# e271828e/Flight.jl

Hardware: AMD Instinct MI355X
Metric: aircraft-steps/sec (higher is better)
Workload: dtype f64

## Files before the change

flight.jl_amd/csrc/c172_duo_device.hpp:

```cpp
#pragma once
#include "c172_device.hpp"

namespace fbd {

#if defined(FB_STAMP) && defined(FB_DUO_TIMELINE)
__device__ unsigned long long g_duo_t0[2];
__device__ __forceinline__ void duo_mark(int role, int k) {
    __builtin_amdgcn_sched_barrier(0);
    if (blockIdx.x == 0 && (threadIdx.x & 255) == 0) {
        const unsigned long long t = __builtin_amdgcn_s_memtime();
        if (k == 0) g_duo_t0[role - 1] = t;
        else if (g_duo_t0[role - 1] != 0) { g_stamp_acc[(role == 1 ? 0 : 16) + k] += t - g_duo_t0[role - 1]; g_stamp_cnt[(role == 1 ? 0 : 16) + k] += 1; }
    }
    __builtin_amdgcn_sched_barrier(0);
}
#define DUO_MARK(role, k) duo_mark(role, k)
#else
#define DUO_MARK(role, k) do { } while (0)
#endif

enum { DUO_PT_T = 0, DUO_PT_V = 1, DUO_PT_X = 2,
       DUO_PT_R = 0, DUO_PT_A = 1, DUO_PT_W = 2,
       DUO_NPT = 3 };
constexpr int XD_FP = 0, XD_TAUP = 3, XD_HROT = 6, XD_RHO = 7, XD_HO = 8, XD_ROWS = 9;
constexpr int XD_VP = XD_FP;
constexpr int DUO_TAP_THETA_ROW = 0, DUO_TAP_WX_ROW = 2, DUO_TAP_VD_ROW = 5, DUO_TAP_EAS_ROW = 7, DUO_TAP_ALPHA_ROW = 8, DUO_TAP_LAT_ROW = 10;

enum {
    KC_P_PROP_HI = KC_HELPERS_END, KC_P_PROP_RSTEP,
    KC_P_WGS_A, KC_P_PROP_RX, KC_P_PROP_RZ,
    KC_P_INV_R, KC_P_INV_SQRT_GR, KC_P_INV_TWO_PI, KC_P_0P1, KC_P_PROP_JXX,
    KC_P_FRC_KP, KC_P_FRC_KI, KC_P_INV_W_IDLE, KC_P_INV_W_RATED, KC_P_INV_P_STD,
    KC_P_N2_LO, KC_P_N2_RSTEP, KC_P_D9_LO, KC_P_D9_RSTEP, KC_P_M9_LO, KC_P_M9_RSTEP,
    KC_P_INV_RHO_STD, KC_P_F_DIFF, KC_P_F_RICH, KC_P_5EM3, KC_P_SQRT_T_STD, KC_P_P_RATED, KC_P_TAU_FRC, KC_P_INV_J, KC_P_INV_M_FUEL,
    KC_P_F_LEAN,
    KC_COUNT
};
FB_KC(KC_P_PROP_HI, 1.5); FB_KC(KC_P_PROP_RSTEP, (PR_NJ - 1) / (1.5 - 0.0));
static_assert(PR_NJ == PR_NM, "one reciprocal step serves both axes of the propeller table");
FB_KC(KC_P_WGS_A, wgs::a); FB_KC(KC_P_PROP_RX, c172::prop_r[0]); FB_KC(KC_P_PROP_RZ, c172::prop_r[2]);
FB_KC(KC_P_INV_R, 1 / isa::R); FB_KC(KC_P_INV_SQRT_GR, 1 / 20.046795704052055); FB_KC_RCP(KC_P_INV_TWO_PI, 2 * PI); FB_KC(KC_P_0P1, 0.1);
FB_KC(KC_P_PROP_JXX, c172::prop_Jxx); FB_KC(KC_P_FRC_KP, 5.0); FB_KC(KC_P_FRC_KI, 200.0);
FB_KC_RCP(KC_P_INV_W_IDLE, c172::w_idle); FB_KC_RCP(KC_P_INV_W_RATED, c172::w_rated); FB_KC_RCP(KC_P_INV_P_STD, isa::p_std);
FB_KC(KC_P_N2_LO, 0.667); FB_KC(KC_P_N2_RSTEP, (2 - 1) / (1.0 - 0.667));
FB_KC(KC_P_D9_LO, 0.441); FB_KC(KC_P_D9_RSTEP, (9 - 1) / (1.0 - 0.441));
FB_KC(KC_P_M9_LO, 0.401); FB_KC(KC_P_M9_RSTEP, (9 - 1) / (0.936 - 0.401));
FB_KC(KC_P_INV_RHO_STD, 1 / isa::rho_std); FB_KC(KC_P_F_DIFF, c172::f_rich - c172::f_lean); FB_KC(KC_P_F_RICH, c172::f_rich); FB_KC(KC_P_5EM3, 5e-3);
FB_KC(KC_P_SQRT_T_STD, isa_sqrt_T_std); FB_KC(KC_P_P_RATED, c172::P_rated); FB_KC(KC_P_TAU_FRC, 0.01 * c172::P_rated / c172::w_rated);
FB_KC_RCP(KC_P_INV_J, c172::J_eng + c172::prop_Jxx); FB_KC_RCP(KC_P_INV_M_FUEL, c172::m_full - c172::m_res);
FB_KC(KC_P_F_LEAN, c172::f_lean);

template <int KIN, int ROLE, class In, class Emit, class XV, class KP = KLit>
__device__ __forceinline__ int32_t rhs_duo(const XV& x, int stall, int eng_state, const In& in, const Env& env, const Tables& T, const Emit& emit, StepAux& aux,
                                           const KP& K = KP{}) {
    using namespace c172;
    static_assert(ROLE == 1 || ROLE == 2, "role P or role D");
    static_assert(KIN == FB_KIN_WA || KIN == FB_KIN_ECEF || KIN == FB_KIN_NED, "kinematic mechanisation");
    int32_t st = 0;
    constexpr int KX = FB_X_Q_WB;
    constexpr bool X = Emit::x2;
    auto gkp = [&](int off) -> gk_cptr { return T.gk + off; };
    auto atan2m = [&](double y, double x0) -> double { return atan2_step(y, x0, T.rk + LDS_ATAN, K); };
    auto atan2p = [&](double y, double x0) -> double { return atan2_step<true>(y, x0, T.rk + LDS_ATAN, K); };

    const double h_e = x[KIN == FB_KIN_WA ? KX + 8 : (KIN == FB_KIN_ECEF ? KX + 7 : KX + 5)];
    if (!(h_e >= H_MIN)) st |= FB_ST_ALT_RANGE;
    [[maybe_unused]] quat q_ew = {1, 0, 0, 0};
    [[maybe_unused]] double dq12 = 0, dq13 = 0, dq24 = 0, dq34 = 0;
    [[maybe_unused]] double ned_cla = 1, pos0 = 0, pos1 = 0, pos2 = 0;
    v3 n_e;
    if constexpr (KIN == FB_KIN_WA) {
        q_ew = {x[KX + 4], x[KX + 5], x[KX + 6], x[KX + 7]};
        dq12 = 2 * q_ew.w * q_ew.x; dq13 = 2 * q_ew.w * q_ew.y;
        dq24 = 2 * q_ew.x * q_ew.z; dq34 = 2 * q_ew.y * q_ew.z;
        n_e = {-(dq24 + dq13), -(dq34 - dq12), -(1 - 2 * (q_ew.x * q_ew.x + q_ew.y * q_ew.y))};
    } else if constexpr (KIN == FB_KIN_ECEF) {
        pos0 = x[KX + 4]; pos1 = x[KX + 5]; pos2 = x[KX + 6];
        n_e = {pos0, pos1, pos2};
    } else {
        pos0 = x[KX + 3]; pos1 = x[KX + 4];
        double sla, slo, clo;
        sincos_step(pos0, sla, ned_cla); sincos_step(pos1, slo, clo);
        n_e = {ned_cla * clo, ned_cla * slo, sla};
    }
    const v3 r_p = {prop_r[0], prop_r[1], prop_r[2]};

    if constexpr (ROLE == 1) {
        lds_cptr PT = T.lds + LDS_PISTON;
        lds_cptr RPT = T.rk + LDS_PISTON;
        const double w_eng = x[FB_X_ENG_OMEGA];
        const double x_frc = x[FB_X_ENG_FRC], x_idle = x[FB_X_ENG_IDLE], x_fuel = x[FB_X_FUEL];
        {
            double pin_w = w_eng, pin_f = x_frc, pin_i = x_idle, pin_u = x_fuel, pin_h = h_e;
            asm volatile("" : "+v"(pin_w), "+v"(pin_f), "+v"(pin_i), "+v"(pin_u), "+v"(pin_h));
            if constexpr (KIN == FB_KIN_WA) {
                double pin_q0 = q_ew.w, pin_q1 = q_ew.x, pin_q2 = q_ew.y, pin_q3 = q_ew.z;
                asm volatile("" : "+v"(pin_q0), "+v"(pin_q1), "+v"(pin_q2), "+v"(pin_q3));
            } else {
                double pin_p0 = pos0, pin_p1 = pos1, pin_p2 = pos2;
                asm volatile("" : "+v"(pin_p0), "+v"(pin_p1), "+v"(pin_p2));
            }
        }
        emit.xpub(DUO_PT_R);
        if constexpr (X) __builtin_amdgcn_s_setprio(0);
        double lat, lon;
        const double h_o = h_e - geoid_height<true>(T, n_e, lat, lon, K);
        if (!(h_o >= H_MIN)) st |= FB_ST_ALT_RANGE;
        if constexpr (X) {
            if (emit.tap) {
                const double ll[2] = {KIN == FB_KIN_NED ? pos0 : lat, KIN == FB_KIN_NED ? pos1 : lon};
                emit.template tap_rows<2>(DUO_TAP_LAT_ROW, ll);
            }
        }
        DUO_MARK(1, 1);
        double T_air, p_air, lnp_air;
        const double h_gp = h_o * kc<KC_P_WGS_A>(K) / (kc<KC_P_WGS_A>(K) + h_o);
        isa_data<true>(h_gp, env.T_sl, env.p_sl, T_air, p_air, lnp_air, st, K);
        const double rs_T = rsqrt(T_air), i_T = rs_T * rs_T;
        const double rho = (p_air * kc<KC_P_INV_R>(K)) * i_T;
        const double i_a_snd = kc<KC_P_INV_SQRT_GR>(K) * rs_T;
        DUO_MARK(1, 2);
        emit.xput(XD_RHO, rho); emit.xput(XD_HO, h_o);
        DUO_MARK(1, 11);
        emit.xpub(DUO_PT_A);
        emit.xwait(DUO_PT_V);
        DUO_MARK(1, 3);

        const double w_prop = w_eng;
        const v3 v_p = {emit.xget(XD_VP), emit.xget(XD_VP + 1), emit.xget(XD_VP + 2)};
        const double v_J = norm(v_p, K);
        const double J_adv = kc<KC_TWO_PI>(K) * v_J / (fmax(fabs(w_prop), 1.0) * prop_d);
        const double Mt = fabs(w_prop) * (prop_d / 2) * i_a_snd;
        const loc lj = range_locate(0.0, kc<KC_P_PROP_HI>(K), kc<KC_P_PROP_RSTEP>(K), PR_NJ, J_adv, true);
        const loc lm = range_locate(0.0, kc<KC_P_PROP_HI>(K), kc<KC_P_PROP_RSTEP>(K), PR_NM, Mt, true);
        const double w00 = (1 - lj.w) * (1 - lm.w), w01 = (1 - lj.w) * lm.w, w10 = lj.w * (1 - lm.w), w11 = lj.w * lm.w;
        gk_cptr g00 = T.gk + LDS_PROP + (lj.i + PR_NJ * lm.i) * PR_NC;
        auto coef = [&](int cidx) {
            return (w00 * g00[cidx] + w01 * g00[PR_NJ * PR_NC + cidx]) + (w10 * g00[PR_NC + cidx] + w11 * g00[PR_NJ * PR_NC + PR_NC + cidx]);
        };
        const double C_Fx = coef(0), C_Mx = coef(1), C_Fz_a = coef(2), C_Mz_a = coef(3);
        double a_p = 0, b_p = 0;
        if (!(v_J < kc<KC_P_0P1>(K))) {
            a_p = atan2m(v_p.z, v_p.x);
            b_p = atan2p(v_p.y, sqrt(v_p.x * v_p.x + v_p.z * v_p.z, K));
        }
// ... 219 lines not shown
        v3 d_e;
        const v3 g_c_c = gravity_com(q_eb, r_bc, n_e, h_e, R_N, R_E, i_RN, i_RE, st, d_e);
        const v3 w_ie_b = earth_rate_b(q_eb);

        DUO_MARK(2, 7);
        emit.xwait(DUO_PT_A);
        const double rho = emit.xget(XD_RHO), h_o = emit.xget(XD_HO);
        if (!(h_o >= H_MIN)) st |= FB_ST_ALT_RANGE;
        if (!(h_o * wgs::a < 84852.0 * (wgs::a + h_o))) st |= FB_ST_ISA_RANGE;
        const double q_dyn = 0.5 * rho * (TAS * TAS);
        if constexpr (X) { if (emit.tap) { const double e1[1] = {TAS * sqrt(rho / isa::rho_std)}; emit.template tap_rows<1>(DUO_TAP_EAS_ROW, e1); } }
        const double p_nd = w_wb_b.x * b * i2V, q_nd = w_wb_b.y * c * i2V, r_nd = w_wb_b.z * b * i2V;
        const double dh_nd = (h_o - env.h_trn) / b;
        const loc l_ge = grid_locate<13, true, AUX_GE>(A + AT_GE_K, RA + AT_GE_K, dh_nd, true, true, gkp(LDS_AERO + AT_GE_K), T.gk);
        auto S_ = [&](int k) -> double { return T.gk[LDS_AERO + AT_SCALARS + k]; };
        if constexpr (X) {
            ac.cy_in = S_(AS_CY_DR) * x2_dr + S_(AS_CY_DA) * x2_da;
            ac.cl_in = S_(AS_CL_DE) * x2_de;
            ac.croll_in = S_(AS_Cl_DA) * x2_da + S_(AS_Cl_DR) * x2_dr;
            ac.cn_in = S_(AS_CN_DR) * x2_dr + S_(AS_CN_DA) * x2_da;
        }
        const double C_D = ac.cd_in + lerp1(A + AT_CD_GE_V, l_ge) * cd_al + cd_be;
        const double C_Y = ac.cy_in + cy_be + cy_p * p_nd + cy_r * r_nd;
        const double C_L = lerp1(A + AT_CL_GE_V, l_ge) * cl_al + ac.cl_in + S_(AS_CL_Q) * q_nd + S_(AS_CL_ALPHA_DOT) * ad_nd;
        const double C_l = ac.croll_in + S_(AS_Cl_BETA) * be + S_(AS_Cl_P) * p_nd + cl_r * r_nd;
        const double C_m = ac.cm_in + S_(AS_CM_ALPHA) * al + S_(AS_CM_Q) * q_nd + S_(AS_CM_ALPHA_DOT) * ad_nd;
        const double C_n = ac.cn_in + S_(AS_CN_BETA) * be + S_(AS_CN_P) * p_nd + S_(AS_CN_R) * r_nd;
        const double qS = q_dyn * S;
        const v3 F_s = {qS * -C_D, qS * C_Y, qS * -C_L};
        const v3 F_a = {cos_al * F_s.x - sin_al * F_s.z, F_s.y, sin_al * F_s.x + cos_al * F_s.z};
        const v3 tau_a = {qS * (C_l * b), qS * (C_m * c), qS * (C_n * b)};
        aux.alpha = alpha;
        aux.wow = 0;
        aux.crash = 0;
        if (!(fmin(h_o - env.h_trn, h_e - H_MIN) > 10.0)) st |= FB_ST_INTERNAL_REDO;
        auto Jmul = [&](v3 v) { return v3{Jxx * v.x + Jxy * v.y + Jxz * v.z, Jxy * v.x + Jyy * v.y + Jyz * v.z, Jxz * v.x + Jyz * v.y + Jzz * v.z}; };
        const v3 v_ec_c = v_eb_b + cross(w_eb_b, r_bc);
        const v3 w_ic_c = w_ie_b + w_eb_b;
        v3 T0 = tau_a - cross(r_bc, F_a) - Jmul(cross(w_ie_b, w_eb_b)) - cross(w_ic_c, Jmul(w_ic_c));
        v3 A0 = iM * F_a + g_c_c - cross(w_eb_b + 2.0 * w_ie_b, v_ec_c);
        const double c11 = Jyy * Jzz - Jyz * Jyz, c12 = Jyz * Jxz - Jxy * Jzz, c13 = Jxy * Jyz - Jyy * Jxz;
        const double c22 = Jxx * Jzz - Jxz * Jxz, c23 = Jxy * Jxz - Jxx * Jyz, c33 = Jxx * Jyy - Jxy * Jxy;
        const double idet = 1 / (Jxx * c11 + Jxy * c12 + Jxz * c13);
        double i11 = c11 * idet, i12 = c12 * idet, i13 = c13 * idet, i22 = c22 * idet, i23 = c23 * idet, i33 = c33 * idet;
        double wy = w_ic_c.y, wz = w_ic_c.z;
        asm volatile("" : "+v"(T0.x), "+v"(T0.y), "+v"(T0.z), "+v"(A0.x), "+v"(A0.y), "+v"(A0.z));
        asm volatile("" : "+v"(i11), "+v"(i12), "+v"(i13), "+v"(i22), "+v"(i23), "+v"(i33), "+v"(wy), "+v"(wz));
        DUO_MARK(2, 8);
        emit.xwait(DUO_PT_W);
        DUO_MARK(2, 9);
        const v3 F_p = {emit.xget(XD_FP), emit.xget(XD_FP + 1), emit.xget(XD_FP + 2)};
        const v3 tau_pb = {emit.xget(XD_TAUP), emit.xget(XD_TAUP + 1), emit.xget(XD_TAUP + 2)};
        const double h_rot = emit.xget(XD_HROT);
        {
            double p0 = F_p.x, p1 = F_p.y, p2 = F_p.z, p3 = tau_pb.x, p4 = tau_pb.y, p5 = tau_pb.z, p6 = h_rot;
            asm volatile("" : "+v"(p0), "+v"(p1), "+v"(p2), "+v"(p3), "+v"(p4), "+v"(p5), "+v"(p6));
        }
        emit.xpub(DUO_PT_X);
        const v3 rw = (T0 + tau_pb) - cross(r_bc, F_p) - v3{0.0, wz * h_rot, -(wy * h_rot)};
        const v3 wd = {i11 * rw.x + i12 * rw.y + i13 * rw.z, i12 * rw.x + i22 * rw.y + i23 * rw.z, i13 * rw.x + i23 * rw.y + i33 * rw.z};
        const v3 vd_b = (A0 + iM * F_p) - cross(wd, r_bc);
        DUO_MARK(2, 10);
        const double kd6[6] = {wd.x, wd.y, wd.z, vd_b.x, vd_b.y, vd_b.z};
        emit_rows<6>(emit, FB_X_OMEGA_EB_B, kd6);
        DUO_MARK(2, 11);
        return st;
    }
}

}
```

flight.jl_amd/csrc/c172_kernels.hpp:

```cpp
#pragma once
#include "c172_device.hpp"
#include "c172x_ctl_device.hpp"
#include "c172_duo_device.hpp"

namespace fbd {

template <bool FAST>
__device__ __forceinline__ void ground_common(quat q_eb, quat q_en, GroundCommon& c) {
    c.q_en = q_en;
    if constexpr (FAST) {
        auto rot_z = [](quat q) { return v3{(2 * q.y) * q.w - (2 * q.z) * (-q.x), (2 * q.z) * q.y - (2 * q.x) * q.w, 1 + ((2 * q.x) * (-q.x) - (2 * q.y) * q.y)}; };
        c.ks_e = rot_z(q_eb);
        c.ut_e = rot_z(c.q_en);
    } else {
        c.ks_e = qrot(q_eb, v3{0, 0, 1});
        c.ut_e = qrot(c.q_en, v3{0, 0, 1});
    }
    c.ut_ks = dot(c.ut_e, c.ks_e);
    if constexpr (FAST) {
        const bool lo = c.ut_ks < 0.5 - 1e-7, hi = c.ut_ks > 0.5 + 1e-7;
        c.tilt_crash = lo;
        if (__builtin_amdgcn_ballot_w64(!lo && !hi) != 0) {
            const double a = acos(fmax(fmin(c.ut_ks, 1.0), -1.0));
            if (!lo && !hi) c.tilt_crash = a * (180 / PI) > 60;
// ... 848 lines not shown
    auto TAP = [&](int k) { return t0[(int64_t)k * n]; };
    auto XS = [&](int k) { return xs[SV::row(k) * B]; };
    CtlIn v;
    {
        const gcptr u0 = (gcptr)(uintptr_t)A.cu + i;
        v.lat = TAP(DUO_TAP_LAT); v.lon = TAP(DUO_TAP_LON); v.EAS = TAP(DUO_TAP_EAS); v.phi = TAP(DUO_TAP_PHI);
        if constexpr (HALF == CTL_HALF_LON) {
            v.theta = TAP(DUO_TAP_THETA); v.clm = -TAP(DUO_TAP_VD); v.alpha = TAP(DUO_TAP_ALPHA);
            v.w_wb_b = {0.0, TAP(DUO_TAP_WY), TAP(DUO_TAP_WZ)};
            v.pos[0] = TAP(DUO_TAP_POS + 0); v.pos[2] = TAP(DUO_TAP_POS + 2); v.cmd[0] = TAP(DUO_TAP_CMD + 0); v.cmd[2] = TAP(DUO_TAP_CMD + 2);
            v.pos[1] = v.pos[3] = v.cmd[1] = v.cmd[3] = 0; v.chi = 0; v.beta = 0;
        } else {
            v.chi = TAP(DUO_TAP_CHI); v.beta = TAP(DUO_TAP_BETA);
            v.theta = 0; v.clm = 0;
            v.w_wb_b = {TAP(DUO_TAP_WX), 0.0, 0.0};
            v.pos[1] = TAP(DUO_TAP_POS + 1); v.pos[3] = TAP(DUO_TAP_POS + 3); v.cmd[1] = TAP(DUO_TAP_CMD + 1); v.cmd[3] = TAP(DUO_TAP_CMD + 3);
            v.pos[0] = v.pos[2] = v.cmd[0] = v.cmd[2] = 0; v.alpha = 0;
        }
#pragma unroll
        for (int k = 0; k < FB_NCU; k++) lu[k] = u0[(int64_t)k * n];
    }
    v.h_e = h_e;
    v.w_eb_b = {XS(FB_X_OMEGA_EB_B), XS(FB_X_OMEGA_EB_B + 1), XS(FB_X_OMEGA_EB_B + 2)};
    v.alpha_filt = XS(FB_X_ALPHA_FILT); v.beta_filt = XS(FB_X_BETA_FILT);
    v.n_eng = XS(FB_X_ENG_OMEGA) / c172::w_rated;
    v.on_gnd = false;
    const CtlMemHalfT<gptr, HALF> M = {(gptr)(uintptr_t)A.cu + i, (gptr)(uintptr_t)A.cs + i, n, lu};
    FB_HALF_STAMP(HALF, HALF == CTL_HALF_LON ? 22 : 16);
    gdc_update(M, v);
    FB_HALF_STAMP(HALF, HALF == CTL_HALF_LON ? 23 : 17);
    const CtlTabT<gcptr> tab = ctl_tab((gcptr)(uintptr_t)A.gains, A.off, v.EAS, v.h_e);
    if constexpr (HALF == CTL_HALF_LON) {
        ctl_lon<true>(tab, M, A.dT, v, (int)M.U(FB_CU_LON_MODE_REQ));
        FB_HALF_STAMP(HALF, 24);
        return {clampd(M.S(FB_CS_THROTTLE_CMD), 0, 1), clampd(M.S(FB_CS_ELEVATOR_CMD), -1, 1)};
    } else {
        const int lat_req = (int)M.U(FB_CU_LAT_MODE_REQ);
        LatGains G;
        G.P = {0, 0, 0, 0};
        ctl_lat<true>(tab, M, A.dT, v, lat_req, G);
        FB_HALF_STAMP(HALF, 19);
        return {clampd(M.S(FB_CS_AILERON_CMD), -1, 1), clampd(M.S(FB_CS_RUDDER_CMD), -1, 1)};
    }
}

constexpr int DUO_B = 256;
constexpr int DUO_NP = 4, DUO_ND = 17;
constexpr int DUO_NPL = 0;
constexpr int DUO_NDL_WA = 13;
constexpr int DUO_NDL_X = 14;
template <int KIN, bool X> constexpr int duo_ndl() { return (KIN == FB_KIN_WA && !X) ? DUO_NDL_WA : (X ? DUO_NDL_X : DUO_ND); }
static_assert(DUO_NDL_WA >= 1 && DUO_NDL_WA <= DUO_ND && DUO_NDL_X >= 1 && DUO_NDL_X <= DUO_ND, "");
template <int KIN, bool X, bool PERENV> constexpr int duo_nk() { return (KIN == FB_KIN_WA && !X && !PERENV) ? (int)KC_COUNT : 0; }
template <int NK>
struct DuoK {
    double r[NK];
    template <int I> static constexpr bool resident() { return I < NK; }
    template <int I> __device__ __forceinline__ double get() const { if constexpr (I < NK) return r[I]; else return KC<I>::v; }
    template <int I = 0> __device__ __forceinline__ void init() {
        if constexpr (I < NK) { double c = KC<I>::v; asm volatile("" : "+v"(c)); r[I] = c; init<I + 1>(); }
    }
};
template <> struct DuoK<0> : KLit { __device__ __forceinline__ void init() {} };
struct InputsDuoP {
    double throttle, mixture;
    int ui;
    __device__ __forceinline__ double get_throttle() const { return throttle; }
    __device__ __forceinline__ double get_mixture() const { return mixture; }
};
struct InputsDuoD {
    static constexpr bool pld_precomputed = true, aero_precomputed = true;
    lds_cptr pld_l;
    const double* aero_g;
    int64_t n;
    int ui;
    __device__ __forceinline__ double get_pld_M() const { return pld_l[0]; }
    __device__ __forceinline__ double get_pld_Mr(int k) const { return pld_l[(1 + k) * DUO_B]; }
    __device__ __forceinline__ double get_pld_J(int k) const { return pld_l[(4 + k) * DUO_B]; }
    static constexpr int SUMS_ROWS = 10;
    __device__ __forceinline__ void fetch_pld_raw(double (&v)[10]) const {
#pragma unroll
        for (int k = 0; k < 10; k++) v[k] = aero_g[(int64_t)k * n];
    }
    __device__ __forceinline__ void fetch_aero(AeroC& c) const {
        double v[DUO_NCONST];
        fetch_aero_raw(v);
        aero_from_raw(v, c);
    }
    __device__ __forceinline__ void fetch_aero_raw(double (&v)[DUO_NCONST]) const {
#pragma unroll
        for (int k = 0; k < DUO_NCONST; k++) v[k] = aero_g[(int64_t)k * n];
    }
    __device__ __forceinline__ static void aero_from_raw(const double (&v)[DUO_NCONST], AeroC& c) {
        c.cd_in = v[0]; c.cd_df = v[1]; c.cy_in = v[2]; c.cl_in = v[3]; c.cl_df = v[4]; c.croll_in = v[5]; c.cm_in = v[6]; c.cn_in = v[7];
        c.l_df4 = {(int)v[8], v[9]}; c.l_df2 = {(int)v[10], v[11]};
    }
};
struct InputsDuoDX : InputsDuoD {
    double pldv[10];
    __device__ __forceinline__ double get_pld_M() const { return pldv[0]; }
    __device__ __forceinline__ double get_pld_Mr(int k) const { return pldv[1 + k]; }
    __device__ __forceinline__ double get_pld_J(int k) const { return pldv[4 + k]; }
};
#ifdef FB_DUO_SYNC_DEBUG
__device__ unsigned g_duo_sync_dbg[40];
#endif
struct DuoSync {
    volatile __attribute__((address_space(3))) int* mine;
    volatile __attribute__((address_space(3))) int* other;
    int base;
    int failed;
};
template <bool GLOBAL = false>
FBD void duo_publish(DuoSync& sy, int k) {
    if constexpr (GLOBAL) asm volatile("s_waitcnt vmcnt(0) lgkmcnt(0)" ::: "memory");
    else asm volatile("s_waitcnt lgkmcnt(0)" ::: "memory");
    *sy.mine = sy.base + k + 1;
    asm volatile("" ::: "memory");
}
FBD void duo_wait(DuoSync& sy, int k) {
#if defined(FB_STAMP) && defined(FB_DUO_WAITPROF)
    const unsigned long long t0 = __builtin_amdgcn_s_memtime();
#endif
    const int c = sy.base + k + 1;
    asm volatile("" ::: "memory");
    int spins = 0;
#pragma unroll 1
    while (__builtin_amdgcn_readfirstlane(*sy.other) < c) {
        __builtin_amdgcn_s_sleep(1);
#ifdef FB_DUO_SYNC_DEBUG
        if (++spins > (1 << 10)) {
            sy.failed = 1;
            if ((threadIdx.x & 63) == 0 && atomicAdd(&g_duo_sync_dbg[0], 1u) < 7) {
                const unsigned q = atomicAdd(&g_duo_sync_dbg[1], 4u);
                g_duo_sync_dbg[2 + q] = blockIdx.x; g_duo_sync_dbg[3 + q] = threadIdx.x; g_duo_sync_dbg[4 + q] = c; g_duo_sync_dbg[5 + q] = *sy.other;
            }
            break;
        }
#else
        if (++spins > (1 << 20)) { sy.failed = 1; break; }
#endif
    }
    asm volatile("" ::: "memory");
#if defined(FB_STAMP) && defined(FB_DUO_WAITPROF)
    const unsigned long long t1 = __builtin_amdgcn_s_memtime();
    if (blockIdx.x == 0 && (threadIdx.x == 0 || threadIdx.x == DUO_B)) {
        const int q = k + (threadIdx.x ? 8 : 0);
        g_stamp_acc[q] += t1 - t0; g_stamp_cnt[q] += 1;
    }
#endif
}

template <int ROLE, bool X = false, int NDL = DUO_ND>
struct DuoEmit {
    static constexpr int role = ROLE;
    static constexpr bool x2 = X;
    typedef void batched_tag;
    using SV = StateLds<DUO_B, false>;
    lds_cptr xs_l;
    lds_ptr xwr_l;
    lds_ptr acc_l;
    double* acc_r;
    lds_ptr xch_l;
    lds_ptr xov_l;
    double eb, ee, em;
    bool last;
    int t;
    DuoSync* sync;
    bool tap;
    int64_t ai;
    const double* xn_r = nullptr;
    template <int N>
    __device__ __forceinline__ void tap_rows(int k0, const double (&v)[N]) const {
        const kargs_cptr ka = kernarg();
        double* const g = ka->duo_tap + ai;
        const int64_t n = ka->n;
#pragma unroll
        for (int e = 0; e < N; e++) g[(int64_t)(k0 + e) * n] = v[e];
    }
    __device__ __forceinline__ static constexpr bool owned(int j) {
        if (SV::skip(j)) return false;
        const int r = SV::row(j);
        return ROLE == 1 ? (r >= 2 && r <= 5) : (r < 2 || r >= 6);
    }
    __device__ __forceinline__ static constexpr int slot(int r) { return ROLE == 1 ? r - 2 : (r < 2 ? r : r - 4); }
    __device__ __forceinline__ double aget(int r) const {
        if (ROLE == 1 && slot(r) >= DUO_NPL) return acc_r[slot(r) - DUO_NPL];
        if (ROLE == 2 && slot(r) >= NDL) return acc_r[slot(r) - NDL];
        return acc_l[slot(r) * DUO_B + t];
    }
    __device__ __forceinline__ void aset(int r, double v) const {
        if (ROLE == 1 && slot(r) >= DUO_NPL) acc_r[slot(r) - DUO_NPL] = v;
        else if (ROLE == 2 && slot(r) >= NDL) acc_r[slot(r) - NDL] = v;
        else acc_l[slot(r) * DUO_B + t] = v;
    }
    __device__ __forceinline__ void operator()(int j, double kj) const {
        static_assert(ROLE == 1 || ROLE == 2, "");
        const int r = SV::row(j), idx = r * DUO_B + t;
        const double xs = (ROLE == 1 && !X) ? xn_r[slot(r)] : xs_l[idx];
        const double A = __builtin_fma(eb, kj, aget(r));
        aset(r, A * em);
        xwr_l[idx] = __builtin_fma(ee, last ? A : kj, xs);
    }
    template <int NE>
    __device__ __forceinline__ void batch(int j0, const double (&k)[NE]) const {
        double xs[NE], A[NE];
#pragma unroll
        for (int e = 0; e < NE; e++) { const int r = SV::row(j0 + e); xs[e] = (ROLE == 1 && !X) ? xn_r[slot(r)] : xs_l[r * DUO_B + t]; A[e] = aget(r); }
#pragma unroll
        for (int e = 0; e < NE; e++) A[e] = __builtin_fma(eb, k[e], A[e]);
#pragma unroll
        for (int e = 0; e < NE; e++) {
            const int r = SV::row(j0 + e);
            aset(r, A[e] * em);
            xwr_l[r * DUO_B + t] = __builtin_fma(ee, last ? A[e] : k[e], xs[e]);
        }
    }
    __device__ __forceinline__ void xput(int k, double v) const { if (k < 6) xov_l[k * DUO_B + t] = v; else xch_l[(k - 6) * DUO_B + t] = v; }
    __device__ __forceinline__ double xget(int k) const { return k < 6 ? xov_l[k * DUO_B + t] : xch_l[(k - 6) * DUO_B + t]; }
    __device__ __forceinline__ void xpub(int k) const { if (X && tap && ROLE == 1) duo_publish<true>(*sync, k); else duo_publish<false>(*sync, k); }
    __device__ __forceinline__ void xwait(int k) const { duo_wait(*sync, k); }
};
constexpr bool duo_rows_ok() {
    int np = 0, nd = 0;
    bool seen_p[DUO_NP] = {}, seen_d[DUO_ND] = {};
    for (int j = 0; j < FB_NX; j++) {
        if (StateLds<DUO_B, false>::skip(j)) { if (DuoEmit<1>::owned(j) || DuoEmit<2>::owned(j)) return false; continue; }
        const int r = StateLds<DUO_B, false>::row(j);
        if (DuoEmit<1>::owned(j) == DuoEmit<2>::owned(j)) return false;
        if (DuoEmit<1>::owned(j)) { const int k = DuoEmit<1>::slot(r); if (k < 0 || k >= DUO_NP || seen_p[k]) return false; seen_p[k] = true; np++; }
        else { const int k = DuoEmit<2>::slot(r); if (k < 0 || k >= DUO_ND || seen_d[k]) return false; seen_d[k] = true; nd++; }
    }
    return np == DUO_NP && nd == DUO_ND;
}
static_assert(duo_rows_ok(), "k_step_duo: row ownership / stage-sum slots");
static_assert(DuoEmit<1>::owned(FB_X_FUEL) && DuoEmit<1>::owned(FB_X_ENG_OMEGA) && DuoEmit<2>::owned(FB_X_Q_WB) && DuoEmit<2>::owned(FB_X_V_EB_B + 2),
              "rhs_duo emits the engine and fuel rows in role P, everything else in role D");
enum { DUO_F_RUN = 1, DUO_F_ZERO_ACC = 2, DUO_F_ENG_SHIFT = 2, DUO_F_CTL = 16 };
enum { DUO_C_EXIT = 4, DUO_C_TAP = 8, DUO_C_CMD = 16 };
constexpr int DUO_PT_U = DUO_NPT, DUO_PT_F = DUO_NPT;
#if defined(FB_STAMP) && defined(FB_DUO_PHASES)
#define DUO_PHASE(k) do { if (blockIdx.x == 0 && threadIdx.x == 256) { __builtin_amdgcn_s_waitcnt(0); g_stamp_acc[8 + (k)] = __builtin_amdgcn_s_memtime(); g_stamp_cnt[8 + (k)] += 1; } } while (0)
#else
#define DUO_PHASE(k) do { } while (0)
#endif
template <int KIN, bool X = false, bool PERENV = false>
__global__ __launch_bounds__(2 * DUO_B) void k_step_duo(KArgs a, int nsteps) {
    constexpr int B = DUO_B, NR = FB_NX - 6, NP = DUO_NP, ND = DUO_ND;
    constexpr int NPT = X ? DUO_NPT + 2 : DUO_NPT;
    constexpr int NAL = FB_ACT_BRAKE_LEFT;
    using SV = StateLds<B, false>;
    __shared__ double lds[AT_SIZE + PT_SIZE];
    __shared__ double rk[LDS_RK_DOUBLES];
    __shared__ double xs_l[NR * B];
    __shared__ double xc_l[NR * B];
    constexpr int DUO_NDL = duo_ndl<KIN, X>();
    __shared__ double accd_l[DUO_NDL * B];
    __shared__ double accp_l[(DUO_NPL > 0 ? DUO_NPL : 1) * B];
    __shared__ double pld_l[10 * B];
    __shared__ double xch_l[(XD_ROWS - 6) * B];
    __shared__ int flags_l[B];
    __shared__ int dst_l[B];
    constexpr bool ENV_LDS = PERENV && (KIN == FB_KIN_WA || X);
    __shared__ double envd_l[ENV_LDS ? 4 * B : 1];
    static_assert(LDS_RK_DOUBLES >= LDS_ATAN + ATAN_N + 2, "room for the control words behind the atan table");
    int* ctrl_l = (int*)&rk[LDS_ATAN + ATAN_N];
// ... 128 lines not shown
            if (c & DUO_C_EXIT) break;
            const bool run = f & DUO_F_RUN;
            const int eng = (f >> DUO_F_ENG_SHIFT) & 3;
            if (f & DUO_F_ZERO_ACC) {
#pragma unroll
                for (int k = 0; k < NP - DUO_NPL; k++) acc_r[k] = 0.0;
#pragma unroll
                for (int k = 0; k < DUO_NPL; k++) accp_l[k * B + t] = 0.0;
            }
            const int stg = c & 3;
            if (!X && stg == 0) {
#pragma unroll
                for (int k = 0; k < NP; k++) xn_r[k] = xs_l[(2 + k) * B + t];
            }
            const StageK sk = stage_k(stg);
            int lds_off = 0;
            asm volatile("" : "+s"(lds_off));
            const Tables T = {(lds_cptr)lds + lds_off, a.egm96, (lds_cptr)rk + lds_off, (gk_cptr)a.tables + lds_off};
            [[maybe_unused]] const bool tap = X && (c & DUO_C_TAP);
            if constexpr (X) { if (sums_for != stg || (c & DUO_C_CMD)) form_sums(stg, lds_off); }
            if (__builtin_amdgcn_ballot_w64(run) != 0) {
                if (run) {
                    StepAux aux;
                    InputsDuoP inl = in;
                    if constexpr (X) {
                        double z = z0;
                        asm volatile("" : "+v"(z));
                        const double ms = act_stage_mc(stg, z);
                        inl.throttle = clampd(act_stage_pos(xa[FB_ACT_THROTTLE], ca[FB_ACT_THROTTLE], ms), 0.0, 1.0);
                    }
                    DUO_MARK(1, 12);
                    asm volatile("" : "+v"(inl.throttle), "+v"(inl.mixture));
                    const DuoEmit<1, X> emit = {(lds_cptr)xs_l, sk.xwr_l, (lds_ptr)accp_l, acc_r, (lds_ptr)xch_l, (lds_ptr)xc_l + 15 * B, sk.eb, sk.ee, sk.em, sk.last, t, &sy,
                                                tap, i, xn_r};
                    if constexpr (X) {
                        if (tap) {
                            static_assert(DUO_TAP_CMD == DUO_TAP_POS + 4, "positions, then commands");
                            const double pc[8] = {clampd(xa[0], 0.0, 1.0), clampd(xa[1], -1.0, 1.0), clampd(xa[2], -1.0, 1.0), clampd(xa[3], -1.0, 1.0), ca[0], ca[1], ca[2], ca[3]};
                            emit.template tap_rows<8>(DUO_TAP_POS, pc);
                        }
                    }
                    const SV xv = {sk.xrd_l + t + lds_off};
#if defined(FB_DUO_ONLY) && FB_DUO_ONLY == 2
                    emit.xpub(DUO_PT_R);
                    emit.xput(XD_RHO, 1.1); emit.xput(XD_HO, 1000.0);
                    emit.xpub(DUO_PT_A);
                    emit.xwait(DUO_PT_V);
                    emit.xput(XD_FP, 900.0); emit.xput(XD_FP + 1, 0.0); emit.xput(XD_FP + 2, 0.0);
                    emit.xput(XD_TAUP, -150.0); emit.xput(XD_TAUP + 1, 0.0); emit.xput(XD_TAUP + 2, 700.0); emit.xput(XD_HROT, 80.0);
                    emit.xpub(DUO_PT_W);
                    emit.xwait(DUO_PT_X);
                    (void)xv; (void)aux; (void)inl;
#else
                    rhs_duo<KIN, 1>(xv, 0, eng, inl, env_p, T, emit, aux, kres);
#endif
                    if constexpr (X) {
                        if (sk.last) {
                            double z = z0;
                            asm volatile("" : "+v"(z));
                            const double P = 1 - z + z * z / 2 - z * z * z / 6 + z * z * z * z / 24;
#pragma unroll
                            for (int k = 0; k < NAL; k++) xa[k] = ca[k] + (xa[k] - ca[k]) * P;
                        }
                    }
                }
            } else duo_publish(sy, DUO_PT_W);
            if constexpr (X) {
                if (tap) {
                    DUO_MARK(1, 13);
                    duo_wait(sy, DUO_PT_U);
                    DUO_MARK(1, 14);
                    const bool ctl = flags_l[t] & DUO_F_CTL;
                    __builtin_amdgcn_s_setprio(X2_LON_PRIO);
#ifdef FB_X2_SKIP_LON
                    if (false) {
#else
                    if (ctl) {
#endif
                        const Ctl2 co = ctl_half(std::integral_constant<int, CTL_HALF_LON>{}, i);
                        ca[FB_ACT_THROTTLE] = co.c0; ca[FB_ACT_ELEVATOR] = co.c1;
                    }
                    DUO_MARK(1, 7);
                    __builtin_amdgcn_s_setprio(0);
                    duo_publish<true>(sy, DUO_PT_F);
                }
                if (tap) sums_for = -1;
                else {
                    __builtin_amdgcn_s_setprio(X2_SPEC_PRIO);
                    form_sums((stg + 1) & 3, lds_off);
                    __builtin_amdgcn_s_setprio(0);
                }
            }
            sy.base += NPT;
        }
        if constexpr (X) {
            const int d = dst_l[t];
            if (valid && (d & D_ACTIVE) && !(d & D_HANDOFF)) {
                bool bad = false;
#pragma unroll
                for (int k = 0; k < NAL; k++) { bad = bad || !isfinite(xa[k]); a.x[(int64_t)(X2_ACT + k) * a.n + i] = xa[k]; }
                if (bad) atomicOr(&a.status[i], (int32_t)FB_ST_NAN);
            }
        }
        if (__builtin_amdgcn_ballot_w64(sy.failed != 0) != 0 && valid) atomicOr(&a.status[i], (int32_t)FB_ST_NAN);
        return;
    }
    InputsDuoD in;
    in.pld_l = (lds_cptr)pld_l + t; in.aero_g = a.duo_pld + (valid ? i : 0); in.n = a.n; in.ui = 0;
    double accd_r[ND > DUO_NDL ? ND - DUO_NDL : 1];
#pragma unroll
    for (int k = 0; k < (ND > DUO_NDL ? ND - DUO_NDL : 1); k++) accd_r[k] = 0.0;
    {
        int stall = 0, eng = 0;
        bool to_ground = false;
        if (valid) {
#pragma unroll
            for (int k = 0; k < FB_NX; k++) {
                const double v = a.x[(int64_t)k * a.n + i];
                if (SV::skip(k)) to_ground = to_ground || (v != 0.0);
                else xs_l[SV::row(k) * B + t] = v;
            }
            if (to_ground) a.redo[i] = 1;
            stall = a.s[i]; eng = a.s[a.n + i];
            DUO_PHASE(5);
            if constexpr (X) {
                InputsXAgg in0;
                in0.xa = nullptr; in0.u_glob = a.u + i; in0.n = a.n; in0.ui = a.ui[i];
                sum_payload_of(in0);
                {
                    const double pv[10] = {in0.pld_M, in0.pld_Mr[0], in0.pld_Mr[1], in0.pld_Mr[2], in0.pld_J[0], in0.pld_J[1], in0.pld_J[2], in0.pld_J[3], in0.pld_J[4], in0.pld_J[5]};
#pragma unroll
                    for (int k = 0; k < 10; k++) a.duo_pld[(int64_t)k * a.n + i] = pv[k];
                }
                in.ui = in0.ui;
                if (a.ctl_ratio > 0 && nsteps > FB_CTL_BAK_SKIP && !to_ground) {
                    copy_rows_batched<FB_NCU, CTL_BAK_G_CU>(a.ctl_bak + (int64_t)FB_NCS * a.n, a.cu, a.n, i);
                }
            } else {
                InputsAgg in0;
                load_inputs(a, i, in0); DUO_PHASE(6); in0.sum_aero((lds_cptr)lds + LDS_AERO, (lds_cptr)rk + LDS_AERO); in0.sum_payload();
                DUO_PHASE(7);
                pld_l[t] = in0.pld_M;
#pragma unroll
                for (int k = 0; k < 3; k++) pld_l[(1 + k) * B + t] = in0.pld_Mr[k];
#pragma unroll
                for (int k = 0; k < 6; k++) pld_l[(4 + k) * B + t] = in0.pld_J[k];
                const double ac[DUO_NCONST] = {in0.cd_in, in0.cd_df, in0.cy_in, in0.cl_in, in0.cl_df, in0.croll_in, in0.cm_in, in0.cn_in,
                                               (double)in0.l_df4.i, in0.l_df4.w, (double)in0.l_df2.i, in0.l_df2.w};
#pragma unroll
                for (int k = 0; k < DUO_NCONST; k++) a.duo_pld[(int64_t)k * a.n + i] = ac[k];
                in.ui = in0.ui;
            }
        }
#pragma unroll
        for (int k = 0; k < DUO_NDL; k++) accd_l[k * B + t] = 0.0;
        const bool active = valid && !to_ground;
        dst_l[t] = (active ? (D_ALIVE | D_ACTIVE) : 0) | (stall ? D_STALL : 0) | (eng << D_ENG_SHIFT);
        flags_l[t] = (active ? DUO_F_RUN : 0) | (eng << DUO_F_ENG_SHIFT);
    }
    DUO_PHASE(2);
    int stage = 0, step = 0;
    bool pending_cb = false, redoing = false, exit_ = __builtin_amdgcn_ballot_w64(dst_l[t] & D_ALIVE) == 0;
    [[maybe_unused]] bool tap_now = false, cmd_put = false;
    if ((threadIdx.x & 63) == 0) ctrl_l[pair] = exit_ ? DUO_C_EXIT : 0;
    __builtin_amdgcn_s_waitcnt(0x0f70);
#pragma unroll 1
    while (true) {
        DUO_MARK(2, 15);
        duo_publish(sy, DUO_PT_T);
        DUO_MARK(2, 0);
        if (exit_) { DUO_PHASE(3); break; }
        const StageK sk = stage_k(stage);
        int lds_off = 0;
        asm volatile("" : "+s"(lds_off));
        const Tables T = {(lds_cptr)lds + lds_off, a.egm96, (lds_cptr)rk + lds_off, (gk_cptr)a.tables + lds_off};
        StepAux aux;
        aux.alpha = 0; aux.m_avail = 0; aux.wow = 0; aux.crash = 0;
        int32_t bits = 0;
        bool run = flags_l[t] & DUO_F_RUN;
        if (__builtin_amdgcn_ballot_w64(run) != 0) {
            if (run) {
                const int d0 = dst_l[t];
                typename std::conditional<X, InputsDuoDX, InputsDuoD>::type inl;
                static_cast<InputsDuoD&>(inl) = in;
                inl.aero_g = in.aero_g + lds_off; inl.pld_l = in.pld_l + lds_off;
                if constexpr (X) {
                    const kargs_cptr ka = kernarg();
                    int64_t il = i;
                    asm volatile("" : "+v"(il));
                    inl.aero_g = ka->duo_pld + il;
                    inl.n = ka->n;
                }
                const DuoEmit<2, X, DUO_NDL> emit = {(lds_cptr)xs_l, sk.xwr_l, (lds_ptr)accd_l, accd_r, (lds_ptr)xch_l, (lds_ptr)xc_l + 15 * B, sk.eb, sk.ee, sk.em, sk.last, t, &sy,
                                            tap_now, i};
                const SV xv = {sk.xrd_l + t + lds_off};
#if defined(FB_DUO_ONLY) && FB_DUO_ONLY == 1
                emit.xput(XD_VP, 50.0); emit.xput(XD_VP + 1, 0.0); emit.xput(XD_VP + 2, 2.0);
                emit.xpub(DUO_PT_V); emit.xwait(DUO_PT_R); emit.xwait(DUO_PT_A); emit.xwait(DUO_PT_W); emit.xpub(DUO_PT_X);
                (void)xv; (void)inl; (void)d0;
#else
                Env env_d = a.env;
                if constexpr (ENV_LDS) {
                    lds_cptr ev = (lds_cptr)envd_l + t + lds_off;
                    env_d.wind_n = ev[0 * B]; env_d.wind_e = ev[1 * B]; env_d.wind_d = ev[2 * B]; env_d.h_trn = ev[3 * B];
                } else if constexpr (PERENV) {
                    const kargs_cptr ka = kernarg();
                    int64_t il = i;
                    asm volatile("" : "+v"(il));
                    const double* e = ka->env_rows + il;
                    const int64_t en = ka->n;
                    env_d.wind_n = e[(int64_t)FB_ENV_WIND_N * en]; env_d.wind_e = e[(int64_t)FB_ENV_WIND_E * en]; env_d.wind_d = e[(int64_t)FB_ENV_WIND_D * en];
                    env_d.h_trn = e[(int64_t)FB_ENV_H_TERRAIN * en];
                }
                bits = rhs_duo<KIN, 2>(xv, (d0 & D_STALL) ? 1 : 0, (d0 >> D_ENG_SHIFT) & 3, inl, env_d, T, emit, aux);
#endif
            }
        } else duo_publish(sy, DUO_PT_X);
        int d = dst_l[t];
        if (run && bits != 0) { d = (d | D_HANDOFF) & ~D_ALIVE; run = false; bits = 0; }
        bool zero_acc = false, advance = true;
        [[maybe_unused]] const bool ctl_now = X && tap_now;
        [[maybe_unused]] const bool ctl_lane = ctl_now && run;
        if (redoing) { redoing = false; run = d & D_ALIVE; }
        else if (stage == 0 && pending_cb) {
            pending_cb = false;
            step++;
            bool mod = false;
            if (run) {
                auto renorm = [&](int k0, int len) {
                    double q[4] = {0, 0, 0, 0}, n2 = 0;
#pragma unroll
                    for (int k = 0; k < 4; k++) if (k < len) { q[k] = xs_l[SV::row(k0 + k) * B + t]; n2 += q[k] * q[k]; }
                    const double nr = ::sqrt(n2);
                    if (fabs(nr - 1.0) > 1e-8) {
#pragma unroll
                        for (int k = 0; k < 4; k++) if (k < len) xs_l[SV::row(k0 + k) * B + t] = q[k] / nr;
                        mod = true;
                    }
                };
                if constexpr (KIN == FB_KIN_WA) { renorm(FB_X_Q_WB, 4); renorm(FB_X_Q_EW, 4); }
                else if constexpr (KIN == FB_KIN_ECEF) { renorm(FB_X_Q_WB, 4); renorm(FB_X_Q_WB + 4, 3); }
                int stall = (d & D_STALL) ? 1 : 0, eng = (d >> D_ENG_SHIFT) & 3;
                const int stall0 = stall, eng0 = eng;
                if (aux.alpha > c172::alpha_stall_hi) stall = 1;
                else if (aux.alpha < c172::alpha_stall_lo) stall = 0;
                const double w = xs_l[SV::row(FB_X_ENG_OMEGA) * B + t];
                const bool fuel = aux.m_avail > 0;
                const bool start = in.ui & FB_UI_ENG_START, stop = in.ui & FB_UI_ENG_STOP;
                if (eng == 0) { if (start) eng = 1; }
                else if (eng == 1) { if (!start) eng = 0; if (w > c172::w_idle && fuel) eng = 2; }
                else if (stop || w < c172::w_stall || !fuel) eng = 0;
                mod = mod || stall != stall0 || eng != eng0;
                d = (d & ~(D_STALL | (3 << D_ENG_SHIFT))) | (stall ? D_STALL : 0) | (eng << D_ENG_SHIFT);
            }
            if (step == nsteps || __builtin_amdgcn_ballot_w64(d & D_ALIVE) == 0) { exit_ = true; advance = false; }
            else if (__builtin_amdgcn_ballot_w64(mod) != 0) {
                if (mod) {
#pragma unroll
                    for (int k = 0; k < DUO_NDL; k++) accd_l[k * B + t] = 0.0;
#pragma unroll
                    for (int k = 0; k < (ND > DUO_NDL ? ND - DUO_NDL : 1); k++) accd_r[k] = 0.0;
                }
                zero_acc = mod; run = mod; redoing = true; advance = false;
            }
        }
        if (advance) {
            stage = (stage + 1) & 3;
            pending_cb = (stage == 0);
        }
        dst_l[t] = d;
        flags_l[t] = (run ? DUO_F_RUN : 0) | (zero_acc ? DUO_F_ZERO_ACC : 0) | (((d >> D_ENG_SHIFT) & 3) << DUO_F_ENG_SHIFT) | (ctl_lane ? DUO_F_CTL : 0);
        if constexpr (X) {
            cmd_put = false;
            if (ctl_now) {
                DUO_MARK(2, 12);
                duo_publish<true>(sy, DUO_PT_U);
                __builtin_amdgcn_s_setprio(X2_UPD_PRIO);
#ifdef FB_X2_SERIAL
                duo_wait(sy, DUO_PT_F);
#endif
#ifdef FB_X2_SKIP_LAT
                if (false) {
#else
                if (ctl_lane) {
#endif
                    const Ctl2 co = ctl_half(std::integral_constant<int, CTL_HALF_LAT>{}, i);
                    xch_l[(XD_RHO - 6) * B + t] = co.c0; xch_l[(XD_HO - 6) * B + t] = co.c1;
                }
                cmd_put = true;
                DUO_MARK(2, 13);
                __builtin_amdgcn_s_setprio(0);
                duo_wait(sy, DUO_PT_F);
                __builtin_amdgcn_s_setprio(DUO_PRIO_D);
                __builtin_amdgcn_s_setprio(DUO_PRIO_D);
                DUO_MARK(2, 14);
            }
            tap_now = a.ctl_ratio > 0 && !exit_ && stage == 0 && pending_cb && !redoing && (a.ctl_phase + step + 1) % a.ctl_ratio == 0;
        }
        if ((threadIdx.x & 63) == 0)
            ctrl_l[pair] = stage | (exit_ ? DUO_C_EXIT : 0) | (tap_now ? DUO_C_TAP : 0) | (cmd_put ? DUO_C_CMD : 0);
        sy.base += NPT;
    }
    const int d = dst_l[t];
    if (!(d & D_ACTIVE)) return;
    if (d & D_HANDOFF) {
        if constexpr (X) {
            if (a.ctl_ratio > 0 && nsteps > FB_CTL_BAK_SKIP) {
#pragma unroll 1
                for (int k = 0; k < FB_NCS; k++) a.cs[(int64_t)k * a.n + i] = a.ctl_bak[(int64_t)k * a.n + i];
#pragma unroll 1
                for (int k = 0; k < FB_NCU; k++) const_cast<double*>(a.cu)[(int64_t)k * a.n + i] = a.ctl_bak[(int64_t)(FB_NCS + k) * a.n + i];
            }
        }
        a.redo[i] = 1;
// ... 580 lines not shown
```

Before: 3.871 billion.

## Pin registers in place, keep register sums, and move aero constants to LDS

For the WA, non-X, shared-env duo path this bundles three changes. Input pin barriers become input-only asm operands, so no copies are made. Register-resident accumulator zeroing moves to the top of the redo iteration and the run-ballot branch becomes unconditional. Seven of the aero constants move from a global SoA buffer into a per-block LDS panel, with the integer indices packed into one double. The aim is to cut VGPR copies, global loads and divergent control flow, at the cost of extra LDS use and a more intricate accumulator-reset protocol.

```diff
diff --git a/flight.jl_amd/csrc/c172_duo_device.hpp b/flight.jl_amd/csrc/c172_duo_device.hpp
--- a/flight.jl_amd/csrc/c172_duo_device.hpp
+++ b/flight.jl_amd/csrc/c172_duo_device.hpp
@@ -50,7 +50,10 @@
 FB_KC_RCP(KC_P_INV_J, c172::J_eng + c172::prop_Jxx); FB_KC_RCP(KC_P_INV_M_FUEL, c172::m_full - c172::m_res);
 FB_KC(KC_P_F_LEAN, c172::f_lean);
 
-template <int KIN, int ROLE, class In, class Emit, class XV, class KP = KLit>
+template <bool PIN_IN_PLACE_ = false>
+struct DuoOpt { static constexpr bool PIN_IN_PLACE = PIN_IN_PLACE_; };
+
+template <int KIN, int ROLE, class OPT = DuoOpt<>, class In, class Emit, class XV, class KP = KLit>
 __device__ __forceinline__ int32_t rhs_duo(const XV& x, int stall, int eng_state, const In& in, const Env& env, const Tables& T, const Emit& emit, StepAux& aux,
                                            const KP& K = KP{}) {
     using namespace c172;
@@ -90,7 +93,11 @@
         lds_cptr RPT = T.rk + LDS_PISTON;
         const double w_eng = x[FB_X_ENG_OMEGA];
         const double x_frc = x[FB_X_ENG_FRC], x_idle = x[FB_X_ENG_IDLE], x_fuel = x[FB_X_FUEL];
-        {
+        if constexpr (OPT::PIN_IN_PLACE) {
+            static_assert(!OPT::PIN_IN_PLACE || KIN == FB_KIN_WA, "PIN_IN_PLACE: the WA mechanisation's position rows");
+            asm volatile("" :: "v"(w_eng), "v"(x_frc), "v"(x_idle), "v"(x_fuel), "v"(h_e));
+            asm volatile("" :: "v"(q_ew.w), "v"(q_ew.x), "v"(q_ew.y), "v"(q_ew.z));
+        } else {
             double pin_w = w_eng, pin_f = x_frc, pin_i = x_idle, pin_u = x_fuel, pin_h = h_e;
             asm volatile("" : "+v"(pin_w), "+v"(pin_f), "+v"(pin_i), "+v"(pin_u), "+v"(pin_h));
             if constexpr (KIN == FB_KIN_WA) {
@@ -416,7 +423,9 @@
         const v3 F_p = {emit.xget(XD_FP), emit.xget(XD_FP + 1), emit.xget(XD_FP + 2)};
         const v3 tau_pb = {emit.xget(XD_TAUP), emit.xget(XD_TAUP + 1), emit.xget(XD_TAUP + 2)};
         const double h_rot = emit.xget(XD_HROT);
-        {
+        if constexpr (OPT::PIN_IN_PLACE) {
+            asm volatile("" :: "v"(F_p.x), "v"(F_p.y), "v"(F_p.z), "v"(tau_pb.x), "v"(tau_pb.y), "v"(tau_pb.z), "v"(h_rot));
+        } else {
             double p0 = F_p.x, p1 = F_p.y, p2 = F_p.z, p3 = tau_pb.x, p4 = tau_pb.y, p5 = tau_pb.z, p6 = h_rot;
             asm volatile("" : "+v"(p0), "+v"(p1), "+v"(p2), "+v"(p3), "+v"(p4), "+v"(p5), "+v"(p6));
         }
diff --git a/flight.jl_amd/csrc/c172_kernels.hpp b/flight.jl_amd/csrc/c172_kernels.hpp
--- a/flight.jl_amd/csrc/c172_kernels.hpp
+++ b/flight.jl_amd/csrc/c172_kernels.hpp
@@ -924,6 +924,14 @@
 template <int KIN, bool X> constexpr int duo_ndl() { return (KIN == FB_KIN_WA && !X) ? DUO_NDL_WA : (X ? DUO_NDL_X : DUO_ND); }
 static_assert(DUO_NDL_WA >= 1 && DUO_NDL_WA <= DUO_ND && DUO_NDL_X >= 1 && DUO_NDL_X <= DUO_ND, "");
 template <int KIN, bool X, bool PERENV> constexpr int duo_nk() { return (KIN == FB_KIN_WA && !X && !PERENV) ? (int)KC_COUNT : 0; }
+constexpr bool DUO_R8_PIN_IN_PLACE = true;
+constexpr bool DUO_R8_SUMS_STAY = true;
+constexpr bool DUO_R8_AERO_PANEL = true;
+template <int KIN, bool X, bool PERENV> constexpr bool duo_r8() { return KIN == FB_KIN_WA && !X && !PERENV; }
+template <bool ALWAYS> __device__ __forceinline__ unsigned long long duo_run_mask(bool run) { if constexpr (ALWAYS) return 1; else return __builtin_amdgcn_ballot_w64(run); }
+template <int KIN, bool X, bool PERENV> constexpr bool duo_sums_stay() { return duo_r8<KIN, X, PERENV>() && DUO_R8_SUMS_STAY; }
+template <int KIN, bool X, bool PERENV> constexpr bool duo_aero_panel() { return duo_r8<KIN, X, PERENV>() && DUO_R8_AERO_PANEL; }
+template <int KIN, bool X, bool PERENV> using duo_opt = DuoOpt<duo_r8<KIN, X, PERENV>() && DUO_R8_PIN_IN_PLACE>;
 template <int NK>
 struct DuoK {
     double r[NK];
@@ -966,6 +974,26 @@
     __device__ __forceinline__ static void aero_from_raw(const double (&v)[DUO_NCONST], AeroC& c) {
         c.cd_in = v[0]; c.cd_df = v[1]; c.cy_in = v[2]; c.cl_in = v[3]; c.cl_df = v[4]; c.croll_in = v[5]; c.cm_in = v[6]; c.cn_in = v[7];
         c.l_df4 = {(int)v[8], v[9]}; c.l_df2 = {(int)v[10], v[11]};
+    }
+};
+struct InputsDuoDL : InputsDuoD {
+    static constexpr int NL = 7, NG = 4;
+    lds_cptr aero_l;
+    __device__ __forceinline__ static void split(const AeroC& c, double (&l)[NL], double (&g)[NG]) {
+        const uint64_t iw = (uint64_t)(uint32_t)c.l_df4.i | ((uint64_t)(uint32_t)c.l_df2.i << 32);
+        l[0] = c.cd_in; l[1] = c.cd_df; l[2] = c.cl_df; l[3] = c.cm_in; l[4] = c.l_df4.w; l[5] = c.l_df2.w; l[6] = __builtin_bit_cast(double, iw);
+        g[0] = c.cy_in; g[1] = c.cl_in; g[2] = c.croll_in; g[3] = c.cn_in;
+    }
+    __device__ __forceinline__ void fetch_aero(AeroC& c) const {
+        double g[NG], l[NL];
+#pragma unroll
+        for (int k = 0; k < NG; k++) g[k] = aero_g[(int64_t)k * n];
+#pragma unroll
+        for (int k = 0; k < NL; k++) l[k] = aero_l[k * DUO_B];
+        const uint64_t iw = __builtin_bit_cast(uint64_t, l[6]);
+        c.cd_in = l[0]; c.cd_df = l[1]; c.cl_df = l[2]; c.cm_in = l[3];
+        c.l_df4 = {(int)(uint32_t)iw, l[4]}; c.l_df2 = {(int)(uint32_t)(iw >> 32), l[5]};
+        c.cy_in = g[0]; c.cl_in = g[1]; c.croll_in = g[2]; c.cn_in = g[3];
     }
 };
 struct InputsDuoDX : InputsDuoD {
@@ -1023,7 +1051,7 @@
 #endif
 }
 
-template <int ROLE, bool X = false, int NDL = DUO_ND>
+template <int ROLE, bool X = false, int NDL = DUO_ND, bool SUMS_STAY = false>
 struct DuoEmit {
     static constexpr int role = ROLE;
     static constexpr bool x2 = X;
@@ -1084,6 +1112,15 @@
 #pragma unroll
         for (int e = 0; e < NE; e++) {
             const int r = SV::row(j0 + e);
+            if constexpr (SUMS_STAY && ROLE == 2) {
+                if (slot(r) >= NDL) {
+                    double sel = last ? A[e] : k[e];
+                    asm volatile("" : "+v"(sel), "+v"(A[e]));
+                    aset(r, A[e] * em);
+                    xwr_l[r * DUO_B + t] = __builtin_fma(ee, sel, xs[e]);
+                    continue;
+                }
+            }
             aset(r, A[e] * em);
             xwr_l[r * DUO_B + t] = __builtin_fma(ee, last ? A[e] : k[e], xs[e]);
         }
@@ -1318,7 +1355,7 @@
                     emit.xwait(DUO_PT_X);
                     (void)xv; (void)aux; (void)inl;
 #else
-                    rhs_duo<KIN, 1>(xv, 0, eng, inl, env_p, T, emit, aux, kres);
+                    rhs_duo<KIN, 1, duo_opt<KIN, X, PERENV>>(xv, 0, eng, inl, env_p, T, emit, aux, kres);
 #endif
                     if constexpr (X) {
                         if (sk.last) {
@@ -1371,8 +1408,12 @@
         if (__builtin_amdgcn_ballot_w64(sy.failed != 0) != 0 && valid) atomicOr(&a.status[i], (int32_t)FB_ST_NAN);
         return;
     }
-    InputsDuoD in;
+    typename std::conditional<duo_aero_panel<KIN, X, PERENV>(), InputsDuoDL, InputsDuoD>::type in;
     in.pld_l = (lds_cptr)pld_l + t; in.aero_g = a.duo_pld + (valid ? i : 0); in.n = a.n; in.ui = 0;
+    if constexpr (duo_aero_panel<KIN, X, PERENV>()) {
+        __shared__ double aero_l[InputsDuoDL::NL * B];
+        in.aero_l = (lds_cptr)aero_l + t;
+    }
     double accd_r[ND > DUO_NDL ? ND - DUO_NDL : 1];
 #pragma unroll
     for (int k = 0; k < (ND > DUO_NDL ? ND - DUO_NDL : 1); k++) accd_r[k] = 0.0;
@@ -1411,10 +1452,23 @@
                 for (int k = 0; k < 3; k++) pld_l[(1 + k) * B + t] = in0.pld_Mr[k];
 #pragma unroll
                 for (int k = 0; k < 6; k++) pld_l[(4 + k) * B + t] = in0.pld_J[k];
+                if constexpr (duo_aero_panel<KIN, X, PERENV>()) {
+                    AeroC c0;
+                    c0.cd_in = in0.cd_in; c0.cd_df = in0.cd_df; c0.cy_in = in0.cy_in; c0.cl_in = in0.cl_in; c0.cl_df = in0.cl_df; c0.croll_in = in0.croll_in;
+                    c0.cm_in = in0.cm_in; c0.cn_in = in0.cn_in; c0.l_df4 = in0.l_df4; c0.l_df2 = in0.l_df2;
+                    double pl[InputsDuoDL::NL], pg[InputsDuoDL::NG];
+                    InputsDuoDL::split(c0, pl, pg);
+                    lds_ptr ap = (lds_ptr)in.aero_l;
+#pragma unroll
+                    for (int k = 0; k < InputsDuoDL::NL; k++) ap[k * B] = pl[k];
+#pragma unroll
+                    for (int k = 0; k < InputsDuoDL::NG; k++) a.duo_pld[(int64_t)k * a.n + i] = pg[k];
+                } else {
                 const double ac[DUO_NCONST] = {in0.cd_in, in0.cd_df, in0.cy_in, in0.cl_in, in0.cl_df, in0.croll_in, in0.cm_in, in0.cn_in,
                                                (double)in0.l_df4.i, in0.l_df4.w, (double)in0.l_df2.i, in0.l_df2.w};
 #pragma unroll
                 for (int k = 0; k < DUO_NCONST; k++) a.duo_pld[(int64_t)k * a.n + i] = ac[k];
+                }
                 in.ui = in0.ui;
             }
         }
@@ -1436,6 +1490,14 @@
         duo_publish(sy, DUO_PT_T);
         DUO_MARK(2, 0);
         if (exit_) { DUO_PHASE(3); break; }
+        if constexpr (duo_sums_stay<KIN, X, PERENV>()) {
+            if (redoing) {
+                if (flags_l[t] & DUO_F_ZERO_ACC) {
+#pragma unroll
+                    for (int k = 0; k < (ND > DUO_NDL ? ND - DUO_NDL : 1); k++) accd_r[k] = 0.0;
+                }
+            }
+        }
         const StageK sk = stage_k(stage);
         int lds_off = 0;
         asm volatile("" : "+s"(lds_off));
@@ -1444,12 +1506,13 @@
         aux.alpha = 0; aux.m_avail = 0; aux.wow = 0; aux.crash = 0;
         int32_t bits = 0;
         bool run = flags_l[t] & DUO_F_RUN;
-        if (__builtin_amdgcn_ballot_w64(run) != 0) {
+        if (duo_run_mask<duo_sums_stay<KIN, X, PERENV>()>(run) != 0) {
             if (run) {
                 const int d0 = dst_l[t];
-                typename std::conditional<X, InputsDuoDX, InputsDuoD>::type inl;
+                typename std::conditional<X, InputsDuoDX, decltype(in)>::type inl;
                 static_cast<InputsDuoD&>(inl) = in;
                 inl.aero_g = in.aero_g + lds_off; inl.pld_l = in.pld_l + lds_off;
+                if constexpr (duo_aero_panel<KIN, X, PERENV>()) inl.aero_l = in.aero_l + lds_off;
                 if constexpr (X) {
                     const kargs_cptr ka = kernarg();
                     int64_t il = i;
@@ -1457,7 +1520,7 @@
                     inl.aero_g = ka->duo_pld + il;
                     inl.n = ka->n;
                 }
-                const DuoEmit<2, X, DUO_NDL> emit = {(lds_cptr)xs_l, sk.xwr_l, (lds_ptr)accd_l, accd_r, (lds_ptr)xch_l, (lds_ptr)xc_l + 15 * B, sk.eb, sk.ee, sk.em, sk.last, t, &sy,
+                const DuoEmit<2, X, DUO_NDL, duo_sums_stay<KIN, X, PERENV>()> emit = {(lds_cptr)xs_l, sk.xwr_l, (lds_ptr)accd_l, accd_r, (lds_ptr)xch_l, (lds_ptr)xc_l + 15 * B, sk.eb, sk.ee, sk.em, sk.last, t, &sy,
                                             tap_now, i};
                 const SV xv = {sk.xrd_l + t + lds_off};
 #if defined(FB_DUO_ONLY) && FB_DUO_ONLY == 1
@@ -1478,10 +1541,11 @@
                     env_d.wind_n = e[(int64_t)FB_ENV_WIND_N * en]; env_d.wind_e = e[(int64_t)FB_ENV_WIND_E * en]; env_d.wind_d = e[(int64_t)FB_ENV_WIND_D * en];
                     env_d.h_trn = e[(int64_t)FB_ENV_H_TERRAIN * en];
                 }
-                bits = rhs_duo<KIN, 2>(xv, (d0 & D_STALL) ? 1 : 0, (d0 >> D_ENG_SHIFT) & 3, inl, env_d, T, emit, aux);
+                bits = rhs_duo<KIN, 2, duo_opt<KIN, X, PERENV>>(xv, (d0 & D_STALL) ? 1 : 0, (d0 >> D_ENG_SHIFT) & 3, inl, env_d, T, emit, aux);
 #endif
             }
         } else duo_publish(sy, DUO_PT_X);
+        if constexpr (duo_sums_stay<KIN, X, PERENV>()) { if (__builtin_amdgcn_ballot_w64(run) == 0) duo_publish(sy, DUO_PT_X); }
         int d = dst_l[t];
         if (run && bits != 0) { d = (d | D_HANDOFF) & ~D_ALIVE; run = false; bits = 0; }
         bool zero_acc = false, advance = true;
@@ -1525,7 +1589,9 @@
 #pragma unroll
                     for (int k = 0; k < DUO_NDL; k++) accd_l[k * B + t] = 0.0;
 #pragma unroll
-                    for (int k = 0; k < (ND > DUO_NDL ? ND - DUO_NDL : 1); k++) accd_r[k] = 0.0;
+                    for (int k = 0; k < (ND > DUO_NDL ? ND - DUO_NDL : 1); k++) {
+                        if constexpr (!(duo_sums_stay<KIN, X, PERENV>())) accd_r[k] = 0.0;
+                    }
                 }
                 zero_acc = mod; run = mod; redoing = true; advance = false;
             }
```

After: 3.962 billion, median of 6. 1.02x the previous value.
